# JohnGBaker/ptmcmc

Hardware: AMD Instinct MI355X
Metric: ladder-wide MH steps/sec (D=32 Gaussian, 1024 temps) (higher is better)
Workload: dtype f64

## Files before the change

### include/ptm_engine.h

```cpp
#ifndef PTM_ENGINE_H
#define PTM_ENGINE_H

#include <stddef.h>
#include <stdint.h>

#ifdef __cplusplus
extern "C" {
#endif

#define PTM_ABI_VERSION 3

typedef struct ptm_engine ptm_engine;

typedef enum {
  PTM_OK = 0,
  PTM_ERR_INVALID = -1,
  PTM_ERR_UNSUPPORTED = -2,
  PTM_ERR_HIP = -3,
  PTM_ERR_NO_DEVICE = -4,
  PTM_ERR_FAR_MOVE = -5,
  PTM_ERR_CALLBACK = -6
} ptm_status;

enum { PTM_BOUND_OPEN = 0, PTM_BOUND_LIMIT = 1, PTM_BOUND_REFLECT = 2, PTM_BOUND_WRAP = 3 };
// ... 137 lines not shown
int ptm_get_history_chains(ptm_engine* e, int chain_begin, int chain_count, double* X, double* llike, double* lprior, int32_t* meta, double* invtemps);
int ptm_set_history(ptm_engine* e, const double* X, const double* llike, const double* lprior, const int32_t* meta,
                    const double* invtemps);
int ptm_set_map(ptm_engine* e, const double* X, const double* lpost, const double* llike, const double* lprior);
int ptm_get_map(ptm_engine* e, double* X, double* lpost, double* llike, double* lprior);
uint64_t ptm_step_count(ptm_engine* e);

int ptm_timer_start(ptm_engine* e);
int ptm_timer_stop(ptm_engine* e, float* elapsed_ms);
int ptm_get_kernel_times(ptm_engine* e, float* ms, int capacity, int* count);
const char* ptm_sweep_kernel_name(ptm_engine* e);
const char* ptm_step_kernel_name(ptm_engine* e);

int ptm_get_ladder_stats(ptm_engine* e, int64_t out[4]);
int ptm_get_counter_sums(ptm_engine* e, int64_t* ntries_sum, int64_t* naccept_sum);
typedef struct ptm_calibration {
  double copy_GBs, copy_bytes, copy_ms;
  double f64_fma_TFs, fma_ms, sclk_MHz;
  int32_t compute_units, reserved;
} ptm_calibration;
int ptm_calibrate(ptm_engine* e, ptm_calibration* out);

int ptm_ess_windowed(ptm_engine* e, int rung, int nfeat, int width, int every, int burn, double* ess , int32_t* nwin );
int ptm_ess_report(ptm_engine* e, int rung, int nfeat, int width, int every, double esslimit, double* ess , int32_t* length );
int ptm_ess_series_windowed(int device, const double* series, int64_t n, int nseries, int nfeat, int width, int every, int burn, double* ess, int32_t* nwin);
int ptm_ess_series_report(int device, const double* series, int64_t n, int nseries, int nfeat, int width, int every, double esslimit, double* ess, int32_t* length);
int ptm_ess_last_on_device(ptm_engine* e);

int ptm_log_evidence(ptm_engine* e, int ilen, double* log_evidence , double* up ,
                     double* down , int32_t* count );
// ... 18 lines not shown
```

### ptmcmc_amd/csrc/ptm_aux_kernels.hpp

```cpp
#pragma once
#include "ptm_kernels.hpp"
#include "ptm_decide.hpp"

namespace ptm {

constexpr int PART_CHUNK = 16384;
__global__ __launch_bounds__(1024) void partition_kernel(int W, int rung0, int nchunk, unsigned char* __restrict__ touch,
                                                         unsigned int* __restrict__ nhist, int* __restrict__ cidx, int* __restrict__ ccnt,
                                                         const unsigned short* __restrict__ rowof) {
  extern __shared__ int plist[];
  __shared__ int wsum[16];
  __shared__ int sbase, stotal;
  const int rl = rung0 + blockIdx.x / nchunk, ch = blockIdx.x % nchunk;
  const int w0 = ch * PART_CHUNK + threadIdx.x * 16;
  const size_t c0 = (size_t)rl * W + w0;
  uint4 v = make_uint4(0x01010101u, 0x01010101u, 0x01010101u, 0x01010101u);
  const bool in = w0 < W;
  if (in) v = *reinterpret_cast<const uint4*>(touch + c0);
  const unsigned int word[4] = {v.x, v.y, v.z, v.w};
  int mine = 0;
  unsigned int zmask = 0, twice = 0;
#pragma unroll
  for (int k = 0; k < 16; ++k) {
    const unsigned int t = (word[k >> 2] >> (8 * (k & 3))) & 0xFFu;
    zmask |= (t == 0u ? 1u : 0u) << k;
    twice |= (t > 1u ? 1u : 0u) << k;
    mine += t == 0u ? 1 : 0;
  }
  int incl = mine;
#pragma unroll
  for (int d = 1; d < 64; d <<= 1) {
    const int up = __shfl_up(incl, d, 64);
    if ((int)(threadIdx.x & 63) >= d) incl += up;
  }
  if ((threadIdx.x & 63) == 63) wsum[threadIdx.x >> 6] = incl;
  __syncthreads();
  if (threadIdx.x == 0) {
    int run = 0;
    for (int k = 0; k < 16; ++k) { const int t = wsum[k]; wsum[k] = run; run += t; }
    stotal = run;
    sbase = run ? atomicAdd(&ccnt[rl], run) : 0;
  }
  __syncthreads();
  if (in) {
    unsigned int slots[8] = {0, 0, 0, 0, 0, 0, 0, 0};
    if (rowof && zmask) {
      const uint4 a = *reinterpret_cast<const uint4*>(rowof + c0), b = *reinterpret_cast<const uint4*>(rowof + c0 + 8);
      slots[0] = a.x; slots[1] = a.y; slots[2] = a.z; slots[3] = a.w; slots[4] = b.x; slots[5] = b.y; slots[6] = b.z; slots[7] = b.w;
    }
    int pos = wsum[threadIdx.x >> 6] + incl - mine;
#pragma unroll
    for (int k = 0; k < 16; ++k)
      if ((zmask >> k) & 1u) plist[pos++] = (w0 + k) | (int)(slots[k >> 1] >> (16 * (k & 1)) << 16);
    if (zmask != 0xFFFFu) *reinterpret_cast<uint4*>(touch + c0) = make_uint4(0, 0, 0, 0);
    if (twice) {
#pragma unroll
      for (int k = 0; k < 16; ++k)
        if ((twice >> k) & 1u) nhist[c0 + k] += ((word[k >> 2] >> (8 * (k & 3))) & 0xFFu) - 1u;
    }
  }
  __syncthreads();
  int* out = cidx + (size_t)rl * W + sbase;
  for (int i = threadIdx.x; i < stotal; i += 1024) out[i] = plist[i];
}
__global__ __launch_bounds__(256) void restore_rows_kernel(double* __restrict__ x, unsigned short* __restrict__ rowof, int W, int Nt, int DP) {
  extern __shared__ unsigned short rr_lds[];
  __shared__ int nlead;
  unsigned short* L = rr_lds;
  unsigned short* lead = rr_lds + Nt;
  const int w = xcd_walker(blockIdx.x, W);
  if (threadIdx.x == 0) nlead = 0;
  for (int r = threadIdx.x; r < Nt; r += 256) L[r] = rowof[(size_t)r * W + w];
  __syncthreads();
  for (int r = threadIdx.x; r < Nt; r += 256) {
    int c = L[r];
    if (c == r) continue;
    int guard = 0;
// ... 308 lines not shown
```

### ptmcmc_amd/csrc/ptm_engine.hip

```cpp
#include <hip/hip_runtime.h>

#include <algorithm>
#include <cmath>
#include <cstddef>
#include <cstdarg>
#include <cstdio>
#include <cstring>
#include <functional>
#include <memory>
#include <string>
#include <vector>

#include "../../include/ptm_engine.h"
#include "ptm_aux_kernels.hpp"
#include "ptm_devlike_kernels.hpp"
#include "ptm_ess_kernels.hpp"
#include "ptm_evidence_kernels.hpp"
#include "ptm_launch.hpp"
#include "ptm_shard_rccl.hpp"

using namespace ptm;

static thread_local std::string g_err;
static int fail(int code, const char* fmt, ...) {
  char buf[512];
  va_list ap;
  va_start(ap, fmt);
  vsnprintf(buf, sizeof buf, fmt, ap);
  va_end(ap);
// ... 70 lines not shown
  void* cb_user = nullptr;
  ptm_logprior_batch_fn prior_cb = nullptr;
  void* prior_user = nullptr;
  ptm_propose_batch_fn pcb = nullptr;
  ptm_proposal_result_fn pres = nullptr;
  void* pcb_user = nullptr;
  ptm_loglike_device_fn dfn = nullptr;
  void* dfn_user = nullptr;
  double *dl_x = nullptr, *dl_ll = nullptr;
  bool dl_own_x = false, dl_own_ll = false;
  int32_t* dl_count = nullptr;
  int *dl_rows = nullptr, *dl_chunks = nullptr;
  double *dl_xprop = nullptr, *dl_lprior_new = nullptr, *dl_llike_new = nullptr, *dl_best = nullptr;
  unsigned char* dl_gate = nullptr;
  int *cidx = nullptr, *ccnt = nullptr;
  bool touched = false;
  bool compact_step = false;
  unsigned short* rowof = nullptr;
  bool rows_labelled = false;
  bool label_step = false;
  ShardComm* shard = nullptr;
  int* shard_ends = nullptr;
  int nshards = 0, halo_nominal = 0;
  int* redo_flag = nullptr;
  long long redo_total = 0;
  double *pub_x = nullptr, *pub_ll = nullptr, *pub_lp = nullptr;
  int *lad_flags = nullptr, *lad_ctl = nullptr;
  long long* lad_prof = nullptr;
  int lad_capacity[2][32] = {{-1, -1, -1, -1, -1, -1, -1, -1, -1, -1, -1, -1, -1, -1, -1, -1, -1, -1, -1, -1, -1, -1, -1, -1, -1, -1, -1, -1, -1, -1, -1, -1},
                             {-1, -1, -1, -1, -1, -1, -1, -1, -1, -1, -1, -1, -1, -1, -1, -1, -1, -1, -1, -1, -1, -1, -1, -1, -1, -1, -1, -1, -1, -1, -1, -1}};
// ... 293 lines not shown

extern "C" int ptm_engine_destroy(ptm_engine* e) {
  if (!e) return PTM_OK;
  (void)ptm_shard_finalize(e);
  (void)hipStreamSynchronize(e->stream);
  {
    std::lock_guard<std::mutex> lock(g_lad_mutex);
    if (g_lad_last == e) g_lad_last = nullptr;
  }
  if (e->lad_event) (void)hipEventDestroy(e->lad_event);
  if (e->shared_handover) e->xprop = e->llike_new = nullptr, e->hastings = nullptr, e->htype = nullptr, e->hvalid = e->acc_out = nullptr;
  if (e->hist_on_host) e->hist.x = e->hist.ll = e->hist.lp = e->hist.beta = nullptr, e->hist.meta = nullptr;
  for (auto& b : e->host_blocks) (void)hipHostFree(b.first);
  void* ptrs[] = {e->xdev, e->rowof, e->ll, e->lp, e->ntries, e->naccept, e->last_type, e->arr_below, e->arr_above, e->mv_src, e->mv_dst, e->mv_n,
                  e->err, e->nhist, e->swap_cnt, e->touch, e->swap_log, e->hist.x, e->hist.ll, e->hist.lp, e->hist.meta, e->map.lpost, e->map.ll, e->map.lp, e->map.x, e->blo,
                  e->bhi, e->ptype, e->bmin, e->bmax, e->plo, e->phi, e->pcoef, e->P2, e->mean, e->beta, e->prop, e->prop_tiles, e->P2_tiles, e->box_row, e->onedfrac, e->mix, e->beta_w, e->betaC, e->beta_add, e->hist.beta, e->xprop, e->lprior_new, e->llike_new, e->hastings, e->htype, e->hvalid, e->acc_out, e->cidx, e->ccnt,
                  e->pub_x, e->lad_flags, e->lad_prof, e->shard_ends, e->redo_flag, e->sums, e->de_init, e->de_hast, e->de_type,
                  e->ada_leaf, e->ada_dbl, e->ada_int, e->dl_own_x ? e->dl_x : nullptr, e->dl_own_ll ? e->dl_ll : nullptr, e->dl_count, e->dl_rows, e->dl_chunks, e->dl_xprop,
                  e->dl_lprior_new, e->dl_llike_new, e->dl_best, e->ess_ws};
  for (void* p : ptrs)
    if (p) (void)hipFree(p);
  if (e->h_sums) (void)hipHostFree(e->h_sums);
  for (hipEvent_t ev : e->kev) (void)hipEventDestroy(ev);
  if (e->t0) (void)hipEventDestroy(e->t0);
  if (e->t1) (void)hipEventDestroy(e->t1);
  if (e->own_stream) (void)hipStreamDestroy(e->stream);
  delete e;
  return PTM_OK;
}

extern "C" int ptm_set_bounds(ptm_engine* e, const int32_t* lo, const int32_t* hi, const double* xmin, const double* xmax) {
  SETTLE(e);
  if (!e || !lo || !hi || !xmin || !xmax) return fail(PTM_ERR_INVALID, "null argument");
  int rc;
  const int D = e->D;
  e->has_bounds = 0;
  e->bounds_box = 1;
// ... 50 lines not shown
        if (a < -M_PI / 2) a = -M_PI / 2;
        if (b > M_PI / 2) b = M_PI / 2;
        coef[d] = std::sin(b) - std::sin(a);
        e->all_uniform = 0;
        break;
      }
      case PTM_PRIOR_LOG:
        if (c[d] <= 0 || h[d] <= 1) return fail(PTM_ERR_INVALID, "log prior needs center>0 and halfwidth>1 (dimension %d)", d);
        lo[d] = c[d] / h[d]; hi[d] = c[d] * h[d]; coef[d] = std::log(hi[d]) - std::log(lo[d]);
        e->all_uniform = 0;
        break;
      default: return fail(PTM_ERR_INVALID, "unknown prior type %d in dimension %d", types[d], d);
    }
  }
  e->lprior_const = std::log(prod);
  e->lp_is_const = false;
  for (int d = 0; d < D; ++d) { e->h_ptype[d] = ty[d]; e->h_plo[d] = lo[d]; e->h_phi[d] = hi[d]; }
  int rc;
  if ((rc = upload(e->ptype, ty.data(), D, e->stream)) || (rc = upload(e->plo, lo.data(), D, e->stream)) ||
      (rc = upload(e->phi, hi.data(), D, e->stream)) || (rc = upload(e->pcoef, coef.data(), D, e->stream)))
    return rc;
  if (e->DP == 32 || e->DP == 64 || e->DP == 128) {
    const int bd = e->DP;
    std::vector<double> box(2 * bd);
    for (int d = 0; d < bd; ++d) {
      box[host_row_pos(bd, d)] = d < D ? lo[d] : -INFINITY;
      box[bd + host_row_pos(bd, d)] = d < D ? hi[d] : INFINITY;
    }
    if ((rc = upload(e->box_row, box.data(), 2 * bd, e->stream))) return rc;
  }
// ... 294 lines not shown
                  kind == PTM_PROP_DIAG ? (row == col ? factors[(size_t)r * D + row] : 0.0) : factors[(size_t)r * D * D + (size_t)row * D + col];
          }
      }
    if ((rc = dalloc(&e->prop_tiles, tiles.size())) || (rc = upload(e->prop_tiles, tiles.data(), tiles.size(), e->stream))) return rc;
  }
  std::vector<double> f(nloc, 0.0);
  e->any_oned = 0;
  if (one_d_frac)
    for (int r = 0; r < nloc; ++r) {
      if (one_d_frac[r] < 0 || one_d_frac[r] > 1) return fail(PTM_ERR_INVALID, "oneDfrac must be in [0,1]");
      f[r] = one_d_frac[r];
      if (f[r] > 0) e->any_oned = 1;
    }
  if ((rc = upload(e->onedfrac, f.data(), (size_t)nloc, e->stream))) return rc;
  e->prop_kind = kind; e->prop_stride = stride; e->have_prop = 1;
  return PTM_OK;
}

static int ada_off(ptm_engine* e) {
  e->ada_on = false;
  if (!e->ada_leaf && !e->ada_dbl && !e->ada_int) return PTM_OK;
  HIPCHK(hipStreamSynchronize(e->stream));
  if (e->ada_leaf) HIPCHK(hipFree(e->ada_leaf));
  if (e->ada_dbl) HIPCHK(hipFree(e->ada_dbl));
  if (e->ada_int) HIPCHK(hipFree(e->ada_int));
  e->ada_leaf = e->ada_dbl = nullptr;
  e->ada_int = nullptr;
  return PTM_OK;
}

// ... 258 lines not shown
  }
  if (DP == 64 || DP == 128) {
    const int NT = DP / 16, ntile = NT * NT * 4;
    std::vector<double> tiles((size_t)ntile * 64, 0.0);
    for (int t = 0; t < ntile; ++t) {
      const int rt = t % NT, sl = (t / NT) & 3, hb = t / (4 * NT);
      for (int k = 0; k < 4; ++k)
        for (int i = 0; i < 16; ++i) {
          const int row = 16 * rt + i, col = 16 * hb + 4 * k + sl;
          if (row < D && col < D)
            tiles[(size_t)t * 64 + 16 * k + i] = kind == PTM_PROP_DIAG ? (row == col ? factor[row] : 0.0) : factor[(size_t)row * D + col];
        }
    }
    if ((rc = upload(e->prop_tiles + (size_t)local_rung * ntile * 64, tiles.data(), tiles.size(), e->stream))) return rc;
  }
  if (one_d_frac >= 0) {
    if (one_d_frac > 1) return fail(PTM_ERR_INVALID, "oneDfrac must be in [0,1]");
    if ((rc = upload(e->onedfrac + local_rung, &one_d_frac, 1, e->stream))) return rc;
    if (one_d_frac > 0) e->any_oned = 1;
  }
  return PTM_OK;
}

static Dev make_dev(ptm_engine* e, bool labelled = false) {
  Dev p;
  memset(&p, 0, sizeof p);
  p.D = e->D; p.DP = e->DP; p.Nt = e->Nt; p.r0 = e->r0; p.nloc = e->nloc; p.W = e->W; p.Nc = e->Nc; p.w_off = e->cfg.walker_begin;
  p.seed = e->cfg.seed; p.step = e->step; p.add_every_n = e->cfg.add_every_n; p.min_prior = e->cfg.min_prior;
  p.has_bounds = e->has_bounds; p.origin_valid = e->origin_valid; p.bounds_box = e->bounds_box;
  p.blo = e->blo; p.bhi = e->bhi; p.bmin = e->bmin; p.bmax = e->bmax;
// ... 215 lines not shown
  for (size_t k0 = 0; k0 < (size_t)n; k0 += Nc) {
    const size_t m = std::min(Nc, (size_t)n - k0);
    for (size_t k = 0; k < Nc; ++k) memcpy(&rows[k * D], X + (k0 + (k < m ? k : 0)) * D, D * 8);
    const int32_t cnt = (int32_t)m;
    HIPCHK(hipMemcpyAsync(e->dl_x, rows.data(), Nc * D * 8, hipMemcpyHostToDevice, e->stream));
    HIPCHK(hipMemcpyAsync(e->dl_count, &cnt, 4, hipMemcpyHostToDevice, e->stream));
    e->dfn(e->dfn_user, (void*)e->stream, (int)Nc, (int)D, e->dl_x, e->dl_count, e->dl_ll);
    HIPCHK(hipMemcpyAsync(llike + k0, e->dl_ll, m * 8, hipMemcpyDeviceToHost, e->stream));
    HIPCHK(hipStreamSynchronize(e->stream));
  }
  return PTM_OK;
}

#define NO_DEVLIKE(e, name) do { if ((e) && (e)->dfn) return fail(PTM_ERR_UNSUPPORTED, name " with a device likelihood is not built (rung-sharded steps)"); } while (0)

static int launch_sweep(ptm_engine* e, int rung0 = 0, int nr = -1, bool last = true) {
  const bool labelled = e->label_step;
  e->label_step = false;
  Dev p = make_dev(e, labelled);
  if (nr < 0) nr = e->nloc - rung0;
  if (rung0 < 0 || nr < 0 || rung0 + nr > e->nloc) return fail(PTM_ERR_INVALID, "rung range out of the shard");
  p.c_begin = rung0 * e->W; p.c_end = (rung0 + nr) * e->W;
  if ((user_like(e) || e->pcb) && (rung0 != 0 || nr != e->nloc)) return fail(PTM_ERR_UNSUPPORTED, "partial sweeps with a user likelihood (host or device) or host-side proposals are not built");
  auto close_step = [&]() {
    e->step += 1; e->touched = false;
    if (e->compact_step) { e->nhist_pending += 1; e->compact_step = false; }
  };
  if (nr == 0) { if (last) close_step(); return PTM_OK; }
  hipEvent_t ev0 = nullptr, ev1 = nullptr;
  if (e->cfg.time_kernels) {
    if (e->kev_used + 2 > e->kev.size()) {
      for (int k = 0; k < 2; ++k) { hipEvent_t ev; HIPCHK(hipEventCreate(&ev)); e->kev.push_back(ev); }
    }
    ev0 = e->kev[e->kev_used]; ev1 = e->kev[e->kev_used + 1];
    e->kev_used += 2;
  }
  const SweepPlan plan = sweep_plan(e, p.c_end - p.c_begin, e->touched);
  if (e->betaC_stale && !reads_ladder_major_beta(plan)) { int rc = ensure_betaC(e); if (rc) return rc; }
  const bool compact = plan.compacted;
  if (labelled && !(compact && rung0 == 0 && nr == e->nloc)) return fail(PTM_ERR_HIP, "internal: a labelled exchange phase without its compacted sweep");
  if (!compact) { int rc = flush_nhist(e); if (rc) return rc; }
  if (compact) {
    if (!e->cidx) { int rc; if ((rc = dalloc(&e->cidx, (size_t)e->Nc)) || (rc = dalloc(&e->ccnt, (size_t)e->nloc))) return rc; }
    HIPCHK(hipMemsetAsync(e->ccnt + rung0, 0, (size_t)nr * sizeof(int), e->stream));
    const int nchunk = (e->W + PART_CHUNK - 1) / PART_CHUNK;
    hipLaunchKernelGGL(partition_kernel, dim3((unsigned)((size_t)nr * nchunk)), dim3(1024), (size_t)PART_CHUNK * sizeof(int), e->stream, e->W, rung0, nchunk, e->touch, e->nhist,
                       e->cidx, e->ccnt, labelled ? (const unsigned short*)e->rowof : nullptr);
    e->compact_step = true;
    HIPCHK(hipGetLastError());
    p.cidx = e->cidx; p.ccnt = e->ccnt; p.cidx_slot = labelled ? 1 : 0;
  }
  if (ev0) HIPCHK(hipEventRecord(ev0, e->stream));
  const AdaArgs ada = make_ada(e);
  const DpLaunch* dl = dp_launch(e->DP);
  if (!dl) return fail(PTM_ERR_UNSUPPORTED, "dim > 1024 is not built");
  auto launch = [&](const Dev& q) { return dl->sweep(q, plan, e->stream, ada); };

  size_t npick = 0;
  if (e->pcb) {
    const size_t Nc = e->Nc, D = e->D, DP = e->DP;
    HIPCHK(hipMemcpyAsync(e->h_rows.data(), xrows(e), Nc * DP * 8, hipMemcpyDeviceToHost, e->stream));
    HIPCHK(hipMemcpyAsync(e->h_touch.data(), e->touch, Nc, hipMemcpyDeviceToHost, e->stream));
    HIPCHK(hipStreamSynchronize(e->stream));
    e->p_pick.clear();
// ... 1349 lines not shown
  int rc = ladder_settle(e);
  if (rc) return rc;
  if (!e->sums) {
    HIPCHK(hipMalloc((void**)&e->sums, 16));
    HIPCHK(hipHostMalloc((void**)&e->h_sums, 16, hipHostMallocDefault));
  }
  HIPCHK(hipMemsetAsync(e->sums, 0, 16, e->stream));
  hipLaunchKernelGGL(counter_sums_kernel, dim3(1024), dim3(256), 0, e->stream, e->ntries, e->naccept, (size_t)e->Nc, e->sums);
  HIPCHK(hipMemcpyAsync(e->h_sums, e->sums, 16, hipMemcpyDeviceToHost, e->stream));
  HIPCHK(hipStreamSynchronize(e->stream));
  if (ntries_sum) *ntries_sum = (int64_t)e->h_sums[0];
  if (naccept_sum) *naccept_sum = (int64_t)e->h_sums[1];
  return PTM_OK;
}

extern "C" int ptm_calibrate(ptm_engine* e, ptm_calibration* out) {
  SETTLE(e);
  if (!e || !out) return fail(PTM_ERR_INVALID, "null argument");
  NO_BATCH(e, "ptm_calibrate");
  memset(out, 0, sizeof *out);
  hipDeviceProp_t prop;
  HIPCHK(hipGetDeviceProperties(&prop, e->device));
  const int cus = prop.multiProcessorCount;
  out->compute_units = cus;
  hipEvent_t a = nullptr, b = nullptr;
  HIPCHK(hipEventCreate(&a));
  HIPCHK(hipEventCreate(&b));
  const size_t half = (size_t)2400 << 20;
  void *src = nullptr, *dst = nullptr;
  HIPCHK(hipMalloc(&src, half));
// ... 465 lines not shown
```

### ptmcmc_amd/csrc/ptm_sweep_plan.hpp

```cpp
#pragma once
#include <cstddef>
#include <cstdio>
#include <cstdlib>

namespace ptm {

enum { PLAN_DENSE = 0, PLAN_DIAG = 1, PLAN_LOWER = 2 };

struct SweepFacts {
  int DP, W;
  long long chains;
  int nloc;
  int kind;
  bool has_bounds, bounds_box, all_uniform, has_mean, any_oned;
  int mix_K;
  bool evolving;
  bool tracked;
  bool user_like;
  bool host_prop;
  bool de, ada;
  int mode;
  bool touched;
};

struct SweepEnv {
  bool force_valu, compact_ok;
};
inline const SweepEnv& sweep_env() {
  static const SweepEnv v = [] {
    const char* f = getenv("PTM_FORCE_VALU");
    const char* c = getenv("PTM_COMPACT");
    return SweepEnv{f && *f && *f != '0', !(c && *c == '0')};
  }();
  return v;
}

enum SweepFamily { FAM_GENERAL, FAM_LANES, FAM_LANES_ADA, FAM_MFMA32, FAM_MFMA64, FAM_MFMA128 };

struct SweepPlan {
  SweepFamily family;
  int DP, kind;
  bool uni, simple, ada;
  bool gen;
  bool hist;
  int mgen;
  bool ev;
  bool bnd;
  bool compacted;
};
inline bool reads_ladder_major_beta(const SweepPlan& s) { return s.family == FAM_MFMA32 && s.mgen == 0 && s.ev; }

#define PTM_LANES_MAX (1ll << 20)

inline SweepPlan plan_sweep(const SweepFacts& f, const SweepEnv& env) {
  SweepPlan s = {};
  s.DP = f.DP;
  s.kind = f.host_prop ? PLAN_DIAG : f.kind;
  const bool uni = (f.W % 64) == 0;
  const bool ada = f.ada && !f.host_prop;
  const bool box = f.all_uniform && (!f.has_bounds || f.bounds_box);
  const bool recipe = f.has_mean || f.any_oned || f.mix_K != 0;
  const bool plain = !f.has_bounds && f.all_uniform && !recipe && !f.user_like && !ada && !f.evolving && !f.host_prop;
  const bool simple = uni && plain;
  const bool lean_ev = uni && f.evolving && !f.has_bounds && f.all_uniform && !recipe && !f.user_like && !ada && !f.host_prop && !f.tracked;
  const bool mfma_ok = uni && f.mode == 0 && !f.user_like && !f.host_prop && !ada && !env.force_valu;
  const int mk = s.kind == PLAN_DIAG ? PLAN_LOWER : s.kind;

  if (f.DP == 32 && mfma_ok && !f.de) {
    s.family = FAM_MFMA32; s.kind = mk;
    s.compacted = env.compact_ok && f.touched && box && !f.tracked && f.W >= 1024 && f.nloc <= 4096;
    s.hist = f.tracked;
    s.mgen = (simple || lean_ev) ? 0 : !box ? 2 : (s.compacted && !recipe) ? 3 : 1;
    s.ev = !simple && box && f.evolving;
    return s;
  }
  if ((f.DP == 64 || f.DP == 128) && mfma_ok && box && !recipe && !f.tracked) {
    s.family = f.DP == 64 ? FAM_MFMA64 : FAM_MFMA128; s.kind = mk;
    s.bnd = f.has_bounds; s.ev = f.evolving;
    return s;
  }
  const long long lanes = f.chains * f.DP;
  const long long lanes_max = f.DP >= 16 ? PTM_LANES_MAX : 4096ll * f.DP, lanes_max_de = f.DP >= 32 ? (1ll << 21) : (1ll << 19);
  if (f.DP >= 64 || f.host_prop ||
      (!env.force_valu && ((!uni && lanes <= lanes_max) || (uni && f.de && f.DP >= 16 && lanes <= lanes_max_de)))) {
    s.family = ada ? FAM_LANES_ADA : FAM_LANES;
    s.gen = !plain;
    return s;
  }
  s.family = FAM_GENERAL;
  s.uni = uni; s.simple = simple; s.ada = ada;
  return s;
}

inline int format_sweep_name(const SweepPlan& s, char* b, size_t n) {
  const auto tf = [](bool v) { return v ? "true" : "false"; };
  switch (s.family) {
    case FAM_MFMA32: return snprintf(b, n, "sweep_mfma32_kernel<%d, %s, %d, %s, %s>", s.kind, tf(s.hist), s.mgen, tf(s.ev), tf(s.compacted));
    case FAM_MFMA64:
    case FAM_MFMA128: return snprintf(b, n, "sweep_mfma%d_kernel<%d, %s, %s>", s.DP, s.kind, tf(s.bnd), tf(s.ev));
    case FAM_LANES: return snprintf(b, n, "sweep_lanes_kernel<%d, %d, %s>", s.DP, s.kind, tf(s.gen));
    case FAM_LANES_ADA: return snprintf(b, n, "sweep_lanes_ada_kernel<%d, %d>", s.DP, s.kind);
    default: break;
  }
  if (s.ada) return snprintf(b, n, "sweep_kernel<%d, %d, %s, false, true>", s.DP, s.kind, tf(s.uni));
  return snprintf(b, n, "sweep_kernel<%d, %d, %s, %s>", s.DP, s.kind, tf(s.uni), tf(s.simple));
}
// ... 15 lines not shown
```

### ptmcmc_amd/engine.py

```python
import ctypes as C
import os
import sys

import numpy as np

_HERE = os.path.dirname(os.path.abspath(__file__))
LIB_PATH = os.environ.get("PTM_ENGINE_LIB") or os.path.join(_HERE, "libptm_engine.so")

BOUND_OPEN, BOUND_LIMIT, BOUND_REFLECT, BOUND_WRAP = 0, 1, 2, 3
PRIOR_FLAT, PRIOR_UNIFORM, PRIOR_GAUSSIAN, PRIOR_POLAR, PRIOR_COPOLAR, PRIOR_LOG = 0, 1, 2, 3, 4, 5
PROP_DENSE, PROP_DIAG, PROP_LOWER = 0, 1, 2
ARR_LLIKE, ARR_LPRIOR, ARR_LPOST, ARR_NTRIES, ARR_NACCEPT, ARR_LAST_TYPE, ARR_NHIST, ARR_NSIZE, ARR_ROW_LABELS = range(9)
FN_LOG, FN_EXP, FN_SIN_0_PI, FN_COS_HPI, FN_SQRT, FN_DIV, FN_SQRT_RAW = range(7)
PRIOR_NAMES = {"uni": 1, "uniform": 1, "gauss": 2, "gaussian": 2, "pol": 3, "polar": 3, "cpol": 4, "copol": 4, "log": 5}

EXPORTS = [
    "ptm_last_error", "ptm_abi_version", "ptm_device_count", "ptm_engine_create", "ptm_engine_destroy",
    "ptm_set_bounds", "ptm_set_prior", "ptm_set_target_gaussian", "ptm_set_target_callback", "ptm_set_prior_callback", "ptm_set_ladder", "ptm_set_evolve_temps", "ptm_get_invtemps", "ptm_set_invtemps",
    "ptm_set_proposals", "ptm_set_proposal_rung", "ptm_set_proposal_mixture", "ptm_set_proposal_callback", "ptm_set_proposal_de", "ptm_set_proposal_prior_draw", "ptm_set_states", "ptm_init_from_prior", "ptm_init_from_prior_k", "ptm_draw_prior_rows", "ptm_get_history_chains", "ptm_sweep", "ptm_step", "ptm_sync",
    "ptm_copy_llike", "ptm_copy_lprior", "ptm_llike_device_ptr", "ptm_exchange_decide", "ptm_exchange_decide_gathered", "ptm_set_shard_map", "ptm_exchange_redo_count", "ptm_exchange_redo", "ptm_exchange_finish_and_sweep", "ptm_exchange_install", "ptm_sweep_rungs", "ptm_exchange_buffer_doubles", "ptm_exchange_row_capacity", "ptm_shard_unique_id", "ptm_shard_init", "ptm_shard_step", "ptm_shard_finalize", "ptm_get_states", "ptm_batch_begin", "ptm_batch_end",
    "ptm_get_array", "ptm_get_swap_counts", "ptm_get_last_swaps", "ptm_max_swaps_per_step", "ptm_get_history", "ptm_get_history_invtemps", "ptm_set_history", "ptm_set_map", "ptm_get_map", "ptm_restore", "ptm_step_count",
    "ptm_timer_start", "ptm_timer_stop", "ptm_get_kernel_times", "ptm_calibrate", "ptm_get_counter_sums", "ptm_get_ladder_stats", "ptm_sweep_kernel_name", "ptm_step_kernel_name", "ptm_debug_eval",
    "ptm_debug_philox", "ptm_debug_boxmuller", "ptm_debug_sqrt_scan", "ptm_debug_evaluate",
    "ptm_dev_alloc", "ptm_dev_free", "ptm_dev_copy",
    "ptm_set_target_device", "ptm_target_device_rows", "ptm_get_best_evaluated",
    "ptm_set_proposal_adaptive", "ptm_get_proposal_adapt_state", "ptm_set_proposal_adapt_state",
    "ptm_ess_windowed", "ptm_ess_report", "ptm_ess_series_windowed", "ptm_ess_series_report", "ptm_ess_last_on_device",
    "ptm_log_evidence",
]


class PtmConfig(C.Structure):
    _fields_ = [("struct_size", C.c_uint32), ("dim", C.c_int32), ("n_rungs", C.c_int32), ("rung_begin", C.c_int32),
                ("rung_count", C.c_int32), ("n_walkers", C.c_int32), ("seed", C.c_uint64), ("swap_rate", C.c_double),
                ("add_every_n", C.c_int32), ("min_prior", C.c_double), ("device", C.c_int32), ("stream", C.c_void_p),
                ("time_kernels", C.c_int32), ("swap_log_steps", C.c_int32), ("exchange_row_capacity", C.c_int32), ("history_rungs", C.c_int32),
                ("history_capacity", C.c_int32), ("map_rungs", C.c_int32), ("walker_begin", C.c_int32)]


class PtmCalibration(C.Structure):
    _fields_ = [("copy_GBs", C.c_double), ("copy_bytes", C.c_double), ("copy_ms", C.c_double), ("f64_fma_TFs", C.c_double),
                ("fma_ms", C.c_double), ("sclk_MHz", C.c_double), ("compute_units", C.c_int32), ("reserved", C.c_int32)]

# ... 80 lines not shown
    L.ptm_exchange_install.argtypes = [C.c_void_p, C.c_void_p, C.c_void_p]
    L.ptm_sweep_rungs.argtypes = [C.c_void_p, C.c_int, C.c_int, C.c_int]
    L.ptm_get_states.argtypes = [C.c_void_p, _dp]
    if hasattr(L, "ptm_batch_begin"):
        L.ptm_batch_begin.argtypes = [C.c_void_p]
        L.ptm_batch_end.argtypes = [C.c_void_p]
    L.ptm_get_array.argtypes = [C.c_void_p, C.c_int, C.c_void_p]
    L.ptm_get_swap_counts.argtypes = [C.c_void_p, _i64p, _i64p]
    L.ptm_get_last_swaps.argtypes = [C.c_void_p, _i32p, _i32p]
    L.ptm_max_swaps_per_step.argtypes = [C.c_void_p]
    L.ptm_timer_start.argtypes = [C.c_void_p]
    L.ptm_timer_stop.argtypes = [C.c_void_p, C.POINTER(C.c_float)]
    L.ptm_get_kernel_times.argtypes = [C.c_void_p, C.POINTER(C.c_float), C.c_int, C.POINTER(C.c_int)]
    L.ptm_calibrate.argtypes = [C.c_void_p, C.POINTER(PtmCalibration)]
    L.ptm_get_counter_sums.argtypes = [C.c_void_p, _i64p, _i64p]
    L.ptm_get_ladder_stats.argtypes = [C.c_void_p, _i64p]
    L.ptm_debug_eval.argtypes = [C.c_int, C.c_int, _dp, _dp, _dp, C.c_int]
    L.ptm_debug_philox.argtypes = [C.c_int, C.c_uint64, C.c_int, C.c_uint32, C.c_uint64, C.c_uint32, _u32p]
    L.ptm_debug_boxmuller.argtypes = [C.c_int, _u32p, _u32p, _dp, _dp, C.c_int]
    L.ptm_exchange_buffer_doubles.argtypes = [C.c_void_p]
    L.ptm_exchange_row_capacity.argtypes = [C.c_void_p]
    L.ptm_get_history.argtypes = [C.c_void_p, _dp, _dp, _dp, _i32p]
    L.ptm_get_history_invtemps.argtypes = [C.c_void_p, _dp]
    L.ptm_set_history.argtypes = [C.c_void_p, _dp, _dp, _dp, _i32p, _dp]
    L.ptm_set_map.argtypes = [C.c_void_p, _dp, _dp, _dp, _dp]
    L.ptm_get_map.argtypes = [C.c_void_p, _dp, _dp, _dp, _dp]
    L.ptm_set_proposal_rung.argtypes = [C.c_void_p, C.c_int, _dp, C.c_double]
    L.ptm_set_proposal_mixture.argtypes = [C.c_void_p, C.c_int, _dp, _dp, _dp]
    L.ptm_set_proposal_de.argtypes = [C.c_void_p, C.POINTER(PtmDeParams), C.c_int, _dp]
    L.ptm_set_proposal_prior_draw.argtypes = [C.c_void_p, C.c_int]
# ... 626 lines not shown
            return np.zeros(0)
        buf = (C.c_float * capacity)()
        _chk(self.L.ptm_get_kernel_times(self.h, buf, capacity, C.byref(n)))
        return np.array(buf[:min(n.value, capacity)], dtype=np.float64)

    def ladder_stats(self):
        o = (C.c_int64 * 4)()
        _chk(self.L.ptm_get_ladder_stats(self.h, o))
        return dict(launches=o[0], fallbacks=o[1], whole_steps=o[2], disabled=bool(o[3]))

    def counter_sums(self):
        t, a = C.c_int64(), C.c_int64()
        _chk(self.L.ptm_get_counter_sums(self.h, C.byref(t), C.byref(a)))
        return t.value, a.value

    def calibrate(self):
        c = PtmCalibration()
        _chk(self.L.ptm_calibrate(self.h, C.byref(c)))
        return {"copy_GBs": c.copy_GBs, "copy_bytes": c.copy_bytes, "copy_ms": c.copy_ms, "f64_fma_TFs": c.f64_fma_TFs,
                "fma_ms": c.fma_ms, "sclk_MHz": c.sclk_MHz, "compute_units": c.compute_units}

    @property
    def sweep_kernel_name(self):
        return self.L.ptm_sweep_kernel_name(self.h).decode()

    @property
    def step_kernel_name(self):
        return self.L.ptm_step_kernel_name(self.h).decode()
```

Baseline: 9.922 billion.

## Add box prefilter kernel to settle out-of-bounds proposals before the sweep

Adds a prefilter stage for rungs whose proposal widths make out-of-box proposals likely. For those rungs the partition kernel sends walkers to a separate list, and a new kernel regenerates the same Philox/MFMA proposal for the first 16 dimensions. Walkers whose proposal leaves the box are settled as rejected (only ntries is incremented), so the main sweep handles fewer walkers. This costs an extra kernel launch, duplicated RNG and proposal work, and host-side flag computation. Whether it runs depends on the sweep plan and on each rung's estimated out-of-box probability.

```diff
diff --git a/include/ptm_engine.h b/include/ptm_engine.h
--- a/include/ptm_engine.h
+++ b/include/ptm_engine.h
@@ -175,6 +175,7 @@
 
 int ptm_get_ladder_stats(ptm_engine* e, int64_t out[4]);
 int ptm_get_counter_sums(ptm_engine* e, int64_t* ntries_sum, int64_t* naccept_sum);
+int ptm_get_prefilter_counts(ptm_engine* e, int64_t out[4]);
 typedef struct ptm_calibration {
   double copy_GBs, copy_bytes, copy_ms;
   double f64_fma_TFs, fma_ms, sclk_MHz;
diff --git a/ptmcmc_amd/csrc/ptm_aux_kernels.hpp b/ptmcmc_amd/csrc/ptm_aux_kernels.hpp
--- a/ptmcmc_amd/csrc/ptm_aux_kernels.hpp
+++ b/ptmcmc_amd/csrc/ptm_aux_kernels.hpp
@@ -7,11 +7,15 @@
 constexpr int PART_CHUNK = 16384;
 __global__ __launch_bounds__(1024) void partition_kernel(int W, int rung0, int nchunk, unsigned char* __restrict__ touch,
                                                          unsigned int* __restrict__ nhist, int* __restrict__ cidx, int* __restrict__ ccnt,
-                                                         const unsigned short* __restrict__ rowof) {
+                                                         const unsigned short* __restrict__ rowof, const unsigned char* __restrict__ pflag,
+                                                         int* __restrict__ pidx, int* __restrict__ pcnt) {
   extern __shared__ int plist[];
   __shared__ int wsum[16];
   __shared__ int sbase, stotal;
   const int rl = rung0 + blockIdx.x / nchunk, ch = blockIdx.x % nchunk;
+  const bool pre = pflag && pflag[rl];
+  int* const lidx = pre ? pidx : cidx;
+  int* const lcnt = pre ? pcnt : ccnt;
   const int w0 = ch * PART_CHUNK + threadIdx.x * 16;
   const size_t c0 = (size_t)rl * W + w0;
   uint4 v = make_uint4(0x01010101u, 0x01010101u, 0x01010101u, 0x01010101u);
@@ -39,7 +43,7 @@
     int run = 0;
     for (int k = 0; k < 16; ++k) { const int t = wsum[k]; wsum[k] = run; run += t; }
     stotal = run;
-    sbase = run ? atomicAdd(&ccnt[rl], run) : 0;
+    sbase = run ? atomicAdd(&lcnt[rl], run) : 0;
   }
   __syncthreads();
   if (in) {
@@ -60,7 +64,7 @@
     }
   }
   __syncthreads();
-  int* out = cidx + (size_t)rl * W + sbase;
+  int* out = lidx + (size_t)rl * W + sbase;
   for (int i = threadIdx.x; i < stotal; i += 1024) out[i] = plist[i];
 }
 __global__ __launch_bounds__(256) void restore_rows_kernel(double* __restrict__ x, unsigned short* __restrict__ rowof, int W, int Nt, int DP) {
diff --git a/ptmcmc_amd/csrc/ptm_box_prefilter.hpp b/ptmcmc_amd/csrc/ptm_box_prefilter.hpp
--- /dev/null
+++ b/ptmcmc_amd/csrc/ptm_box_prefilter.hpp
@@ -0,0 +1,126 @@
+#pragma once
+#include "ptm_kernels.hpp"
+
+namespace ptm {
+
+struct BoxPre {
+  int W, Nt, r0, w_off;
+  int rung0, nrung;
+  int labelled;
+  uint64_t seed, step;
+  const double* x;
+  const double *ll, *lp;
+  const double* beta;
+  const double* prop_tiles;
+  const double* box_row;
+  int* ntries;
+  const int *pidx, *pcnt;
+  int *cidx, *ccnt;
+  unsigned long long* counts;
+};
+
+typedef double bp_d4 __attribute__((ext_vector_type(4)));
+typedef double bp_d2 __attribute__((ext_vector_type(2)));
+
+inline size_t box_prefilter_lds(int nrung) { return (size_t)(BM_TABLE_DOUBLES + 64) * sizeof(double) + ((size_t)nrung + 260) * sizeof(int); }
+
+__global__ __launch_bounds__(256) void box_prefilter_kernel(const BoxPre p) {
+  extern __shared__ __attribute__((aligned(16))) double bp_lds[];
+  double* lbox = bp_lds + BM_TABLE_DOUBLES;
+  int* tpre = reinterpret_cast<int*>(lbox + 64);
+  const int wave = threadIdx.x >> 6, l = threadIdx.x & 63, q = l >> 4, j = l & 15;
+#pragma unroll
+  for (int t = 0; t < BM_TABLE_DOUBLES / 512; ++t)
+    reinterpret_cast<bm_d2*>(bp_lds)[threadIdx.x + 256 * t] = reinterpret_cast<const bm_d2*>(BM_TABLE)[threadIdx.x + 256 * t];
+  if (threadIdx.x < 64) lbox[threadIdx.x] = p.box_row[threadIdx.x];
+  const int nrung = p.nrung, per = (nrung + 255) / 256;
+  int loc = 0;
+  for (int k = 0; k < per; ++k) {
+    const int r = threadIdx.x * per + k;
+    if (r < nrung) { loc += (p.pcnt[p.rung0 + r] + 255) >> 8; tpre[r] = loc; }
+  }
+  int* tsum = tpre + nrung;
+  tsum[threadIdx.x] = loc;
+  __syncthreads();
+  if (threadIdx.x == 0) { int run = 0; for (int t = 0; t < 256; ++t) { const int v = tsum[t]; tsum[t] = run; run += v; } tsum[256] = run; }
+  __syncthreads();
+  const int off = tsum[threadIdx.x];
+  for (int k = 0; k < per; ++k) {
+    const int r = threadIdx.x * per + k;
+    if (r < nrung) tpre[r] += off;
+  }
+  __syncthreads();
+  const int ntiles = tsum[256];
+  const bp_d2* box = reinterpret_cast<const bp_d2*>(lbox) + q;
+  const int wmask = p.labelled ? 0xFFFF : -1;
+  unsigned int seen = 0, settled = 0;
+  for (int tile = blockIdx.x; tile < ntiles; tile += gridDim.x) {
+    int lo = 0, hi = nrung - 1;
+    while (lo < hi) { const int mid = (lo + hi) >> 1; if (tpre[mid] > tile) hi = mid; else lo = mid + 1; }
+    const int r = __builtin_amdgcn_readfirstlane(lo);
+    const int kb = tile - (r ? tpre[r - 1] : 0);
+    const int rl = p.rung0 + r, rg = p.r0 + rl;
+    const int start = (kb * 4 + wave) * 64, cnt = p.pcnt[rl];
+    if (start >= cnt) continue;
+    const int nact = cnt - start < 64 ? cnt - start : 64;
+    const size_t lbase = (size_t)rl * p.W;
+    const int mine = p.pidx[lbase + start + (l < nact ? l : nact - 1)];
+    const int c = (int)lbase + (mine & wmask);
+    const double ll = p.ll[c], lp = p.lp[c];
+    const double beta = as_c(p.beta)[rg];
+    const double* timg = p.prop_tiles + (size_t)rl * (16 * 64) + l;
+    double ta[4];
+#pragma unroll
+    for (int sl = 0; sl < 4; ++sl) ta[sl] = timg[((0 * 4 + sl) * 2 + 0) * 64];
+    const bp_d2 lo0 = box[0], lo1 = box[4], hi0 = box[16], hi1 = box[20];
+    bp_d2 v0[4], v1[4];
+    int wk[4];
+#pragma unroll
+    for (int g = 0; g < 4; ++g) {
+      const int e = __shfl(mine, 16 * g + j, 64);
+      const int slot = p.labelled ? (int)((unsigned int)e >> 16) : rl;
+      wk[g] = e & wmask;
+      const bp_d2* rp = reinterpret_cast<const bp_d2*>(p.x + ((size_t)slot * p.W + wk[g]) * 32) + q;
+      v0[g] = rp[0];
+      v1[g] = rp[4];
+    }
+    uint64_t inbox = 0;
+#pragma unroll
+    for (int g = 0; g < 4; ++g) {
+      const uint32_t stream = (uint32_t)(wk[g] + p.w_off) * (uint32_t)p.Nt + (uint32_t)rg;
+      const u32x4 o = draw_block(p.seed, TAG_MH, stream, p.step, (uint32_t)(1 + q));
+      double z[4];
+      boxmuller(o.v0, o.v1, (const double*)bp_lds, z[0], z[1]);
+      boxmuller(o.v2, o.v3, (const double*)bp_lds, z[2], z[3]);
+      bp_d4 acc = bp_d4{0.0, 0.0, 0.0, 0.0};
+#pragma unroll
+      for (int sl = 0; sl < 4; ++sl) acc = __builtin_amdgcn_mfma_f64_16x16x4f64(ta[sl], z[sl], acc, 0, 0, 0);
+      const double x0 = v0[g].x + acc[0], x1 = v0[g].y + acc[1], x2 = v1[g].x + acc[2], x3 = v1[g].y + acc[3];
+      const bool ok = !(x0 < lo0.x) & !(x0 > hi0.x) & !(x1 < lo0.y) & !(x1 > hi0.y) & !(x2 < lo1.x) & !(x2 > hi1.x) & !(x3 < lo1.y) & !(x3 > hi1.y);
+      uint64_t b = __builtin_amdgcn_ballot_w64(ok);
+      b &= b >> 32;
+      b &= b >> 16;
+      inbox |= (b & 0xFFFFull) << (16 * g);
+    }
+    const double cur_lpost = lp + beta * ll;
+    const bool live = l < nact;
+    const bool finite = __builtin_fabs(cur_lpost) < __builtin_inf();
+    const bool settle = live && finite && ((inbox >> l) & 1ull) == 0;
+    if (settle) p.ntries[c] += 1;
+    const bool keep = live && !settle;
+    const uint64_t kbits = __builtin_amdgcn_ballot_w64(keep);
+    const int nk = __builtin_popcountll(kbits);
+    int base = 0;
+    if (l == 0 && nk) base = atomicAdd(&p.ccnt[rl], nk);
+    base = __builtin_amdgcn_readfirstlane(base);
+    if (keep) p.cidx[lbase + base + __builtin_popcountll(kbits & ((1ull << l) - 1ull))] = mine;
+    seen += (unsigned int)nact;
+    settled += (unsigned int)(nact - nk);
+  }
+  if (l == 0 && seen) {
+    atomicAdd(p.counts, (unsigned long long)seen);
+    if (settled) atomicAdd(p.counts + 1, (unsigned long long)settled);
+  }
+}
+
+}
diff --git a/ptmcmc_amd/csrc/ptm_engine.hip b/ptmcmc_amd/csrc/ptm_engine.hip
--- a/ptmcmc_amd/csrc/ptm_engine.hip
+++ b/ptmcmc_amd/csrc/ptm_engine.hip
@@ -13,6 +13,7 @@
 
 #include "../../include/ptm_engine.h"
 #include "ptm_aux_kernels.hpp"
+#include "ptm_box_prefilter.hpp"
 #include "ptm_devlike_kernels.hpp"
 #include "ptm_ess_kernels.hpp"
 #include "ptm_evidence_kernels.hpp"
@@ -113,6 +114,12 @@
   double *dl_xprop = nullptr, *dl_lprior_new = nullptr, *dl_llike_new = nullptr, *dl_best = nullptr;
   unsigned char* dl_gate = nullptr;
   int *cidx = nullptr, *ccnt = nullptr;
+  int *pidx = nullptr, *pcnt = nullptr;
+  unsigned char *pf_flag = nullptr, *h_pf_flag = nullptr;
+  unsigned long long* pf_counts = nullptr;
+  std::vector<double> pf_sigma;
+  bool pf_dirty = true;
+  int pf_flagged = 0, pf_grid = 0;
   bool touched = false;
   bool compact_step = false;
   unsigned short* rowof = nullptr;
@@ -436,13 +443,14 @@
   for (auto& b : e->host_blocks) (void)hipHostFree(b.first);
   void* ptrs[] = {e->xdev, e->rowof, e->ll, e->lp, e->ntries, e->naccept, e->last_type, e->arr_below, e->arr_above, e->mv_src, e->mv_dst, e->mv_n,
                   e->err, e->nhist, e->swap_cnt, e->touch, e->swap_log, e->hist.x, e->hist.ll, e->hist.lp, e->hist.meta, e->map.lpost, e->map.ll, e->map.lp, e->map.x, e->blo,
-                  e->bhi, e->ptype, e->bmin, e->bmax, e->plo, e->phi, e->pcoef, e->P2, e->mean, e->beta, e->prop, e->prop_tiles, e->P2_tiles, e->box_row, e->onedfrac, e->mix, e->beta_w, e->betaC, e->beta_add, e->hist.beta, e->xprop, e->lprior_new, e->llike_new, e->hastings, e->htype, e->hvalid, e->acc_out, e->cidx, e->ccnt,
+                  e->bhi, e->ptype, e->bmin, e->bmax, e->plo, e->phi, e->pcoef, e->P2, e->mean, e->beta, e->prop, e->prop_tiles, e->P2_tiles, e->box_row, e->onedfrac, e->mix, e->beta_w, e->betaC, e->beta_add, e->hist.beta, e->xprop, e->lprior_new, e->llike_new, e->hastings, e->htype, e->hvalid, e->acc_out, e->cidx, e->ccnt, e->pidx, e->pcnt, e->pf_flag, e->pf_counts,
                   e->pub_x, e->lad_flags, e->lad_prof, e->shard_ends, e->redo_flag, e->sums, e->de_init, e->de_hast, e->de_type,
                   e->ada_leaf, e->ada_dbl, e->ada_int, e->dl_own_x ? e->dl_x : nullptr, e->dl_own_ll ? e->dl_ll : nullptr, e->dl_count, e->dl_rows, e->dl_chunks, e->dl_xprop,
                   e->dl_lprior_new, e->dl_llike_new, e->dl_best, e->ess_ws};
   for (void* p : ptrs)
     if (p) (void)hipFree(p);
   if (e->h_sums) (void)hipHostFree(e->h_sums);
+  if (e->h_pf_flag) (void)hipHostFree(e->h_pf_flag);
   for (hipEvent_t ev : e->kev) (void)hipEventDestroy(ev);
   if (e->t0) (void)hipEventDestroy(e->t0);
   if (e->t1) (void)hipEventDestroy(e->t1);
@@ -523,6 +531,7 @@
     }
   }
   e->lprior_const = std::log(prod);
+  e->pf_dirty = true;
   e->lp_is_const = false;
   for (int d = 0; d < D; ++d) { e->h_ptype[d] = ty[d]; e->h_plo[d] = lo[d]; e->h_phi[d] = hi[d]; }
   int rc;
@@ -847,6 +856,9 @@
     }
   if ((rc = upload(e->onedfrac, f.data(), (size_t)nloc, e->stream))) return rc;
   e->prop_kind = kind; e->prop_stride = stride; e->have_prop = 1;
+  e->pf_sigma.assign((size_t)nloc * PREFILTER_DIMS, 0.0);
+  for (int r = 0; r < nloc; ++r) prefilter_sigmas(kind == PTM_PROP_DIAG, factors + (size_t)r * (kind == PTM_PROP_DIAG ? D : D * D), D, &e->pf_sigma[(size_t)r * PREFILTER_DIMS]);
+  e->pf_dirty = true;
   return PTM_OK;
 }
 
@@ -1135,6 +1147,8 @@
     }
     if ((rc = upload(e->prop_tiles + (size_t)local_rung * ntile * 64, tiles.data(), tiles.size(), e->stream))) return rc;
   }
+  prefilter_sigmas(kind == PTM_PROP_DIAG, factor, D, &e->pf_sigma[(size_t)local_rung * PREFILTER_DIMS]);
+  e->pf_dirty = true;
   if (one_d_frac >= 0) {
     if (one_d_frac > 1) return fail(PTM_ERR_INVALID, "oneDfrac must be in [0,1]");
     if ((rc = upload(e->onedfrac + local_rung, &one_d_frac, 1, e->stream))) return rc;
@@ -1380,6 +1394,22 @@
 
 #define NO_DEVLIKE(e, name) do { if ((e) && (e)->dfn) return fail(PTM_ERR_UNSUPPORTED, name " with a device likelihood is not built (rung-sharded steps)"); } while (0)
 
+static int prefilter_flags(ptm_engine* e) {
+  const int nd = e->D < PREFILTER_DIMS ? e->D : PREFILTER_DIMS;
+  double width[PREFILTER_DIMS];
+  for (int d = 0; d < nd; ++d) width[d] = e->h_phi[d] - e->h_plo[d];
+  if (!e->h_pf_flag) HIPCHK(hipHostMalloc((void**)&e->h_pf_flag, (size_t)e->nloc, hipHostMallocDefault));
+  unsigned char* fl = e->h_pf_flag;
+  e->pf_flagged = 0;
+  for (int r = 0; r < e->nloc; ++r) {
+    fl[r] = (e->pf_sigma.size() == (size_t)e->nloc * PREFILTER_DIMS && prefilter_flag(&e->pf_sigma[(size_t)r * PREFILTER_DIMS], width, nd, sweep_env().prefilter)) ? 1 : 0;
+    e->pf_flagged += fl[r];
+  }
+  HIPCHK(hipMemcpyAsync(e->pf_flag, fl, (size_t)e->nloc, hipMemcpyHostToDevice, e->stream));
+  e->pf_dirty = false;
+  return PTM_OK;
+}
+
 static int launch_sweep(ptm_engine* e, int rung0 = 0, int nr = -1, bool last = true) {
   const bool labelled = e->label_step;
   e->label_step = false;
@@ -1409,11 +1439,43 @@
   if (compact) {
     if (!e->cidx) { int rc; if ((rc = dalloc(&e->cidx, (size_t)e->Nc)) || (rc = dalloc(&e->ccnt, (size_t)e->nloc))) return rc; }
     HIPCHK(hipMemsetAsync(e->ccnt + rung0, 0, (size_t)nr * sizeof(int), e->stream));
+    bool pre = plan.prefilter;
+    if (pre) {
+      if (!e->pidx) {
+        int rc;
+        if ((rc = dalloc(&e->pidx, (size_t)e->Nc)) || (rc = dalloc(&e->pcnt, (size_t)e->nloc)) || (rc = dalloc(&e->pf_flag, (size_t)e->nloc)) || (rc = dalloc(&e->pf_counts, 2))) return rc;
+        HIPCHK(hipMemsetAsync(e->pf_counts, 0, 16, e->stream));
+        e->pf_dirty = true;
+      }
+      if (e->pf_dirty) { int rc = prefilter_flags(e); if (rc) return rc; }
+      pre = e->pf_flagged > 0;
+      if (pre) HIPCHK(hipMemsetAsync(e->pcnt + rung0, 0, (size_t)nr * sizeof(int), e->stream));
+    }
     const int nchunk = (e->W + PART_CHUNK - 1) / PART_CHUNK;
     hipLaunchKernelGGL(partition_kernel, dim3((unsigned)((size_t)nr * nchunk)), dim3(1024), (size_t)PART_CHUNK * sizeof(int), e->stream, e->W, rung0, nchunk, e->touch, e->nhist,
-                       e->cidx, e->ccnt, labelled ? (const unsigned short*)e->rowof : nullptr);
+                       e->cidx, e->ccnt, labelled ? (const unsigned short*)e->rowof : nullptr, pre ? (const unsigned char*)e->pf_flag : nullptr, e->pidx, e->pcnt);
     e->compact_step = true;
     HIPCHK(hipGetLastError());
+    if (pre) {
+      BoxPre b;
+      memset(&b, 0, sizeof b);
+      b.W = e->W; b.Nt = e->Nt; b.r0 = e->r0; b.w_off = e->cfg.walker_begin; b.rung0 = rung0; b.nrung = nr; b.labelled = labelled ? 1 : 0;
+      b.seed = e->cfg.seed; b.step = e->step;
+      b.x = p.x; b.ll = e->ll; b.lp = e->lp; b.beta = e->beta; b.prop_tiles = e->prop_tiles; b.box_row = e->box_row; b.ntries = e->ntries;
+      b.pidx = e->pidx; b.pcnt = e->pcnt; b.cidx = e->cidx; b.ccnt = e->ccnt; b.counts = e->pf_counts;
+      const size_t lds = box_prefilter_lds(nr);
+      if (!e->pf_grid) {
+        int per_cu = 0, dev = 0;
+        hipDeviceProp_t pr;
+        if (hipOccupancyMaxActiveBlocksPerMultiprocessor(&per_cu, (const void*)box_prefilter_kernel, 256, box_prefilter_lds(e->nloc)) != hipSuccess || per_cu <= 0) { (void)hipGetLastError(); per_cu = 2; }
+        HIPCHK(hipGetDevice(&dev));
+        HIPCHK(hipGetDeviceProperties(&pr, dev));
+        e->pf_grid = per_cu * (pr.multiProcessorCount > 0 ? pr.multiProcessorCount : 256);
+      }
+      const long long tiles = (long long)nr * ((e->W + 255) / 256);
+      hipLaunchKernelGGL(box_prefilter_kernel, dim3((unsigned)(tiles < e->pf_grid ? tiles : e->pf_grid)), dim3(256), lds, e->stream, b);
+      HIPCHK(hipGetLastError());
+    }
     p.cidx = e->cidx; p.ccnt = e->ccnt; p.cidx_slot = labelled ? 1 : 0;
   }
   if (ev0) HIPCHK(hipEventRecord(ev0, e->stream));
@@ -2793,6 +2855,21 @@
   return PTM_OK;
 }
 
+extern "C" int ptm_get_prefilter_counts(ptm_engine* e, int64_t out[4]) {
+  if (!e || !out) return fail(PTM_ERR_INVALID, "null argument");
+  NO_BATCH(e, "ptm_get_prefilter_counts");
+  int rc = ladder_settle(e);
+  if (rc) return rc;
+  out[0] = out[1] = out[2] = 0;
+  out[3] = step_sweep_plan(e).prefilter ? 1 : 0;
+  if (!e->pf_counts) return PTM_OK;
+  unsigned long long h[2];
+  HIPCHK(hipMemcpyAsync(h, e->pf_counts, 16, hipMemcpyDeviceToHost, e->stream));
+  HIPCHK(hipStreamSynchronize(e->stream));
+  out[0] = (int64_t)h[0]; out[1] = (int64_t)h[1]; out[2] = e->pf_flagged;
+  return PTM_OK;
+}
+
 extern "C" int ptm_calibrate(ptm_engine* e, ptm_calibration* out) {
   SETTLE(e);
   if (!e || !out) return fail(PTM_ERR_INVALID, "null argument");
diff --git a/ptmcmc_amd/csrc/ptm_sweep_plan.hpp b/ptmcmc_amd/csrc/ptm_sweep_plan.hpp
--- a/ptmcmc_amd/csrc/ptm_sweep_plan.hpp
+++ b/ptmcmc_amd/csrc/ptm_sweep_plan.hpp
@@ -1,4 +1,5 @@
 #pragma once
+#include <cmath>
 #include <cstddef>
 #include <cstdio>
 #include <cstdlib>
@@ -25,12 +26,14 @@
 
 struct SweepEnv {
   bool force_valu, compact_ok;
+  int prefilter;
 };
 inline const SweepEnv& sweep_env() {
   static const SweepEnv v = [] {
     const char* f = getenv("PTM_FORCE_VALU");
     const char* c = getenv("PTM_COMPACT");
-    return SweepEnv{f && *f && *f != '0', !(c && *c == '0')};
+    const char* b = getenv("PTM_BOX_PREFILTER");
+    return SweepEnv{f && *f && *f != '0', !(c && *c == '0'), (b && *b) ? (*b == '0' ? -1 : 1) : 0};
   }();
   return v;
 }
@@ -47,6 +50,7 @@
   bool ev;
   bool bnd;
   bool compacted;
+  bool prefilter;
 };
 inline bool reads_ladder_major_beta(const SweepPlan& s) { return s.family == FAM_MFMA32 && s.mgen == 0 && s.ev; }
 
@@ -72,6 +76,7 @@
     s.hist = f.tracked;
     s.mgen = (simple || lean_ev) ? 0 : !box ? 2 : (s.compacted && !recipe) ? 3 : 1;
     s.ev = !simple && box && f.evolving;
+    s.prefilter = env.prefilter >= 0 && s.compacted && s.mgen == 0 && !s.ev && (f.kind == PLAN_LOWER || f.kind == PLAN_DIAG);
     return s;
   }
   if ((f.DP == 64 || f.DP == 128) && mfma_ok && box && !recipe && !f.tracked) {
@@ -90,6 +95,38 @@
   s.family = FAM_GENERAL;
   s.uni = uni; s.simple = simple; s.ada = ada;
   return s;
+}
+
+constexpr int PREFILTER_DIMS = 16;
+#ifndef PTM_PREFILTER_THRESHOLD
+#define PTM_PREFILTER_THRESHOLD 0.70
+#endif
+inline void prefilter_sigmas(bool diag, const double* factor, int D, double* sigma) {
+  for (int d = 0; d < PREFILTER_DIMS; ++d) {
+    double s2 = 0.0;
+    if (d < D) {
+      if (diag) s2 = factor[d] * factor[d];
+      else for (int k = 0; k < D; ++k) s2 += factor[(size_t)d * D + k] * factor[(size_t)d * D + k];
+    }
+    sigma[d] = std::sqrt(s2);
+  }
+}
+inline double prefilter_out_1d(double sigma, double w) {
+  if (!(sigma > 0.0) || !(w < INFINITY)) return 0.0;
+  if (!(w > 0.0)) return 1.0;
+  const double u = w / sigma, phi0 = 0.3989422804014327;
+  const double in = std::erf(u * 0.7071067811865476) - (2.0 / u) * (phi0 - phi0 * std::exp(-0.5 * u * u));
+  return in < 0.0 ? 1.0 : (in > 1.0 ? 0.0 : 1.0 - in);
+}
+inline double prefilter_out_share(const double* sigma, const double* width, int nd) {
+  double in = 1.0;
+  for (int d = 0; d < nd; ++d) in *= 1.0 - prefilter_out_1d(sigma[d], width[d]);
+  return 1.0 - in;
+}
+inline bool prefilter_flag(const double* sigma, const double* width, int nd, int env_prefilter) {
+  if (env_prefilter < 0) return false;
+  if (env_prefilter > 0) return true;
+  return prefilter_out_share(sigma, width, nd) > PTM_PREFILTER_THRESHOLD;
 }
 
 inline int format_sweep_name(const SweepPlan& s, char* b, size_t n) {
diff --git a/ptmcmc_amd/engine.py b/ptmcmc_amd/engine.py
--- a/ptmcmc_amd/engine.py
+++ b/ptmcmc_amd/engine.py
@@ -27,6 +27,7 @@
     "ptm_set_proposal_adaptive", "ptm_get_proposal_adapt_state", "ptm_set_proposal_adapt_state",
     "ptm_ess_windowed", "ptm_ess_report", "ptm_ess_series_windowed", "ptm_ess_series_report", "ptm_ess_last_on_device",
     "ptm_log_evidence",
+    "ptm_get_prefilter_counts",
 ]
 
 
@@ -137,6 +138,8 @@
     L.ptm_get_kernel_times.argtypes = [C.c_void_p, C.POINTER(C.c_float), C.c_int, C.POINTER(C.c_int)]
     L.ptm_calibrate.argtypes = [C.c_void_p, C.POINTER(PtmCalibration)]
     L.ptm_get_counter_sums.argtypes = [C.c_void_p, _i64p, _i64p]
+    if hasattr(L, "ptm_get_prefilter_counts"):
+        L.ptm_get_prefilter_counts.argtypes = [C.c_void_p, _i64p]
     L.ptm_get_ladder_stats.argtypes = [C.c_void_p, _i64p]
     L.ptm_debug_eval.argtypes = [C.c_int, C.c_int, _dp, _dp, _dp, C.c_int]
     L.ptm_debug_philox.argtypes = [C.c_int, C.c_uint64, C.c_int, C.c_uint32, C.c_uint64, C.c_uint32, _u32p]
@@ -793,6 +796,11 @@
         _chk(self.L.ptm_get_counter_sums(self.h, C.byref(t), C.byref(a)))
         return t.value, a.value
 
+    def prefilter_counts(self):
+        o = (C.c_int64 * 4)()
+        _chk(self.L.ptm_get_prefilter_counts(self.h, o))
+        return dict(seen=o[0], settled=o[1], rungs_flagged=o[2], eligible=bool(o[3]))
+
     def calibrate(self):
         c = PtmCalibration()
         _chk(self.L.ptm_calibrate(self.h, C.byref(c)))
```

Measured after the change: 10.79 billion (median of 6 runs). 1.09x the previous value.
